# BlaineHeffron/WaveformML

Hardware: AMD Instinct MI355X
Metric: waveforms/sec (LitPSD sparse-conv training step) (higher is better)
Workload: dtype bf16; 1 GPU; SubMConv3d PSD net, 14x11 PMT grid x 256 samples, Cin=2 Cout=32, 256 events/rank/step, rulebook rebuilt every step; active_voxels_per_rank=84164, global_batch=256, parallelism=dp1, execution=hipgraph

## Files before the change

### include/wfsparse.h

```cpp
#ifndef WFSPARSE_H
#define WFSPARSE_H

#include <stddef.h>
#include <stdint.h>

#ifdef __cplusplus
extern "C" {
#endif

#define WFS_OK 0
#define WFS_EINVAL 1
#define WFS_EOVERFLOW 2
#define WFS_EHIP 3
#define WFS_EWORKSPACE 4

#define WFS_F32 0
#define WFS_BF16 1
#define WFS_F16 2

#define WFS_MAX_DIM 4

#define WFS_ABI_VERSION 6
int wfs_abi_version(void);
const char *wfs_last_error(void);
// ... 86 lines not shown
    int32_t transpose;
    float *dW;
} wfs_dw_job;

int wfs_gather_dw(const int32_t *table, const int32_t *kmap_host, int32_t K, int32_t identity_k,
                  int64_t R, const void *S, int32_t Cs, const void *G, int64_t G_rows, int32_t Cg,
                  int32_t swap, float *dW, int32_t dtype, void *workspace, size_t workspace_bytes,
                  const int64_t *r_dev, wfs_dw_job *defer, int32_t packed_kl, void *stream);

int wfs_conv_backward(const int32_t *table, int32_t K, int32_t identity_k, int64_t R, const void *X, const void *dY,
                      int64_t dY_rows, int32_t Cin, int32_t Cout, const float *W, void *dX, float *dW, int32_t dtype,
                      void *workspace, size_t workspace_bytes, const int64_t *r_dev, wfs_dw_job *defer,
                      int32_t packed_kl, void *stream);

int wfs_dw_reduce_jobs(const wfs_dw_job *jobs, int32_t n, void *stream);

size_t wfs_column_sum_workspace_bytes(int32_t C);
int wfs_column_sum(const void *X, int64_t R, int32_t C, float *out, void *workspace, size_t workspace_bytes,
                   int32_t dtype, const int64_t *r_dev, void *stream);

int wfs_scatter_conv(const int32_t *table, int32_t K, int32_t identity_k, int64_t R, const void *X,
                     int32_t Cx, const float *W, int32_t Cw_in, int32_t Cw_out, int32_t transpose_w,
                     float *Y_accum, int32_t dtype, void *stream);

int wfs_maxpool_fwd(const int32_t *table, const int32_t *kmap_host, int32_t K, int64_t R, const void *X, int64_t X_rows,
                    int32_t C, void *Y, int32_t dtype, const int64_t *r_dev, void *stream);
int wfs_maxpool_packed_ok(int32_t packed_kl, int32_t K, int32_t C, int32_t dtype);
int wfs_maxpool_bwd(const int32_t *table, int32_t K, int32_t packed_kl, int64_t N, const void *X, const void *Y,
                    const void *dY, int64_t M_rows, int32_t C, void *dX, int32_t dtype, const int64_t *n_dev, void *stream);

// ... 289 lines not shown
```

### waveformml_amd/_lib.py

```python
import ctypes
import os

import torch

_HERE = os.path.dirname(os.path.abspath(__file__))
LIB_PATH = os.environ.get("WFS_LIB") or os.path.join(_HERE, "lib", "libwfsparse.so")

WFS_OK, WFS_EINVAL, WFS_EOVERFLOW, WFS_EHIP, WFS_EWORKSPACE = 0, 1, 2, 3, 4
WFS_F32, WFS_BF16, WFS_F16 = 0, 1, 2
WFS_TENSOR_TARGET_I64 = 3
WFS_MAX_DIM = 4
WFS_RNN_RELU, WFS_RNN_TANH = 0, 1
WFS_LOSS_L1, WFS_LOSS_MSE = 0, 1
WFS_PREDICT_ROWS_PER_BLOCK = 256
WFS_PREDICT_WAVEFORM, WFS_PREDICT_PULSE = 0, 1
WFS_PREDICT_DENSE, WFS_PREDICT_EVENT, WFS_PREDICT_ROWS = 0, 1, 2
WFS_ABI_VERSION = 6
TIMER_GATHER_CONV, TIMER_GATHER_DW, TIMER_RULEBOOK, TIMER_CONV_BACKWARD = 0, 1, 2, 3

c_i32p = ctypes.POINTER(ctypes.c_int32)
c_i64p = ctypes.POINTER(ctypes.c_int64)
c_f32p = ctypes.POINTER(ctypes.c_float)
_vp, _i32, _i64, _sz = ctypes.c_void_p, ctypes.c_int32, ctypes.c_int64, ctypes.c_size_t
_dbl = ctypes.c_double
# ... 41 lines not shown
    "wfs_wide_linear_ok": (ctypes.c_int, [_i64, _i32, _i32, _i32]),
    "wfs_wide_linear_workspace_bytes": (_sz, [_i64, _i32, _i32, _i32]),
    "wfs_wide_linear_fwd": (ctypes.c_int, [_vp, _i64, _i32, _vp, _vp, _i32, _vp, _i32, _vp, _sz, _vp]),
    "wfs_wide_linear_bwd": (ctypes.c_int, [_vp, _vp, _i64, _i32, _vp, _i32, _vp, _vp, _vp, _i32, _vp, _sz, _vp]),
    "wfs_event_offsets_ints": (_sz, [_i32]),
    "wfs_event_offsets": (ctypes.c_int, [_vp, _i64, _i32, _i32, _vp, _vp, _vp]),
    "wfs_event_rulebook_ok": (ctypes.c_int, [ctypes.POINTER(Geometry)]),
    "wfs_event_rulebook_flag_ints": (_sz, [_i32]),
    "wfs_event_rulebook_subm": (ctypes.c_int, [ctypes.POINTER(Geometry), _vp, _i64, _vp, _vp, _vp, _vp, _vp, _vp]),
    "wfs_gather_dw_workspace_bytes": (_sz, [_i32, _i64, _i32, _i32]),
    "wfs_gather_dw": (ctypes.c_int, [_vp, c_i32p, _i32, _i32, _i64, _vp, _i32, _vp, _i64, _i32, _i32, _vp, _i32, _vp,
                                     _sz, _vp, ctypes.POINTER(DwJob), _i32, _vp]),
    "wfs_conv_backward": (ctypes.c_int, [_vp, _i32, _i32, _i64, _vp, _vp, _i64, _i32, _i32, _vp, _vp, _vp, _i32, _vp, _sz,
                                         _vp, ctypes.POINTER(DwJob), _i32, _vp]),
    "wfs_dw_reduce_jobs": (ctypes.c_int, [ctypes.POINTER(DwJob), _i32, _vp]),
    "wfs_scatter_conv": (ctypes.c_int, [_vp, _i32, _i32, _i64, _vp, _i32, _vp, _i32, _i32, _i32, _vp, _i32, _vp]),
    "wfs_maxpool_fwd": (ctypes.c_int, [_vp, c_i32p, _i32, _i64, _vp, _i64, _i32, _vp, _i32, _vp, _vp]),
    "wfs_maxpool_packed_ok": (ctypes.c_int, [_i32, _i32, _i32, _i32]),
    "wfs_maxpool_bwd": (ctypes.c_int, [_vp, _i32, _i32, _i64, _vp, _vp, _vp, _i64, _i32, _vp, _i32, _vp, _vp]),
    "wfs_bn_workspace_bytes": (_sz, [_i64, _i32]),
    "wfs_column_sum_workspace_bytes": (_sz, [_i32]),
    "wfs_column_sum": (ctypes.c_int, [_vp, _i64, _i32, _vp, _vp, _sz, _i32, _vp, _vp]),
    "wfs_bn_relu_fwd": (ctypes.c_int, [_vp, _i64, _i32, _vp, _vp, _vp, _vp, _vp, ctypes.c_float, ctypes.c_float, _i32,
                                       _i32, _vp, _vp, _vp, _vp, _sz, _i32, _vp, _vp]),
    "wfs_bn_relu_bwd": (ctypes.c_int, [_vp, _vp, _i64, _i32, _vp, _vp, _vp, _vp, _i32, _i32, _vp, _vp, _vp, _vp, _sz,
                                       _i32, _vp, _vp]),
    "wfs_rulebook_cell_map": (ctypes.c_int, [ctypes.POINTER(Geometry), _i64, _vp, ctypes.POINTER(_vp), ctypes.POINTER(_vp),
                                             c_i64p]),
    "wfs_to_dense_mapped": (ctypes.c_int, [_vp, _vp, _vp, _i64, _vp, _i32, _i64, _i32, _vp, _i32, _vp]),
    "wfs_to_dense_bwd_mapped": (ctypes.c_int, [_vp, _vp, _vp, _i64, _vp, _i32, _i64, _i32, _vp, _i32, _vp]),
# ... 192 lines not shown
```

### waveformml_amd/csrc/bn.hip

```cpp
#include "wfs_common.h"

#include <atomic>
#include <cstdlib>
#include <mutex>

namespace {

constexpr int TB = 256;
constexpr int MAXC = 1024;

__device__ __forceinline__ long long valid_rows(long long N, const long long *n_dev) {
    long long v = n_dev ? *n_dev : N;
    return v < N ? v : N;
}

template <typename T, int VEC>
__device__ __forceinline__ void load_vec(const T *p, float *out) {
    if constexpr (VEC == 4 && sizeof(T) == 4) {
        float4 v = *reinterpret_cast<const float4 *>(p);
        out[0] = v.x; out[1] = v.y; out[2] = v.z; out[3] = v.w;
    } else if constexpr (VEC == 4) {
        uint2 v = *reinterpret_cast<const uint2 *>(p);
        wfs_unpack2<T>(v.x, out[0], out[1]);
        wfs_unpack2<T>(v.y, out[2], out[3]);
// ... 964 lines not shown
                                                              (int)nblk, save_mean, save_invstd, gamma, beta,       \
                                                              training, relu, (T *)dX, dgamma, dbeta);              \
    } while (0)
    if (dtype == WFS_F32) {
        if (vec4) WFS_BN_BWD(float, 4); else WFS_BN_BWD(float, 1);
    } else if (dtype == WFS_BF16) {
        if (vec4) WFS_BN_BWD(wfs_bf16, 4); else WFS_BN_BWD(wfs_bf16, 1);
    } else {
        if (vec4) WFS_BN_BWD(wfs_f16, 4); else WFS_BN_BWD(wfs_f16, 1);
    }
#undef WFS_BN_BWD
    WFS_LAUNCH_CHECK();
    return WFS_OK;
}

extern "C" int wfs_bn_relu_bwd(const void *X, const void *dY, int64_t N, int32_t C, const float *gamma,
                               const float *beta, const float *save_mean, const float *save_invstd, int32_t training,
                               int32_t relu, void *dX, float *dgamma, float *dbeta, void *workspace,
                               size_t workspace_bytes, int32_t dtype, const int64_t *n_dev_, void *stream_) {
    hipStream_t stream = (hipStream_t)stream_;
    const long long *n_dev = (const long long *)n_dev_;
    if (bw_ok(N, C) && N > 0 && wfs_dtype_ok(dtype)) {
        WFS_REQUIRE(X && dY && dX && save_mean && save_invstd && workspace, WFS_EINVAL, "NULL device pointer");
        WFS_REQUIRE(workspace_bytes >= wfs_bn_workspace_bytes(N, C), WFS_EWORKSPACE, "workspace too small");
        float *partial = (float *)workspace;
        if (dtype == WFS_F32)
            return bw_bwd<float>(X, dY, N, C, gamma, beta, save_mean, save_invstd, training, relu, dX, dgamma, dbeta,
                                 partial, n_dev, stream);
        if (dtype == WFS_BF16)
            return bw_bwd<wfs_bf16>(X, dY, N, C, gamma, beta, save_mean, save_invstd, training, relu, dX, dgamma, dbeta,
// ... 23 lines not shown
```

### waveformml_amd/csrc/conv_mfma.hip

```cpp
#include <stdlib.h>

#include "wfs_common.h"

namespace {

typedef float f32x16 __attribute__((ext_vector_type(16)));
typedef float f32x4 __attribute__((ext_vector_type(4)));
constexpr int F32_GROUP = 4;

struct KMap {
    int v[128];
};

__device__ __forceinline__ long long valid_rows(long long R, const long long *r_dev) {
    long long v = r_dev ? *r_dev : R;
    return v < R ? v : R;
}

__device__ __forceinline__ int packed_entry(int e, int o) { return (e >= 0 && (e & 7) == o) ? (e >> 3) : -1; }
__device__ __forceinline__ void table_row_of(int pk, int k, int *trow, int *osel) {
    const int kq = pk ? k / pk : k;
    *trow = kq;
    *osel = pk ? k - kq * pk : -1;
}
// ... 1151 lines not shown
            int col = (i & 3) + 8 * (i >> 2) + 4 * h;
            sRed[wid * 1024 + col * 32 + c] = half ? acc1[i] : acc0[i];
        }
        __syncthreads();
        for (int e = threadIdx.x; e < 1024; e += 512) {
            float v = 0.f;
#pragma unroll
            for (int w = 0; w < C2_WAVES; ++w) v += sRed[w * 1024 + e];
            const int ee = half * 1024 + e;
            if (ee < K * 64) part[(long long)blockIdx.x * K * 64 + ee] = v;
        }
        __syncthreads();
    }
}

constexpr int C2F_WAVES = 8;
__global__ void __launch_bounds__(512, 2) k_gdw_c32c2_f32(const int *__restrict__ table, int mirror, int K, int identity_k,
                                                         long long Rcap, const long long *__restrict__ r_dev,
                                                         const float *__restrict__ S, const float *__restrict__ G,
                                                         float *__restrict__ part) {
    __shared__ int sNbT[C2F_WAVES][28 * 33];
    __shared__ float sRed[C2F_WAVES][1024];
    const int lane = threadIdx.x & 63, wid = threadIdx.x >> 6;
    const int c = lane & 31, h = lane >> 5;
    int *myNb = sNbT[wid];
    const long long R = valid_rows(Rcap, r_dev);
    const long long ntiles = (R + 31) >> 5;
    f32x16 acc0, acc1;
#pragma unroll
    for (int i = 0; i < 16; ++i) acc0[i] = acc1[i] = 0.f;
// ... 523 lines not shown
                table, mirror, K, identity_k, R, r_dev, (const wfs_bf16 *)S, (const wfs_bf16 *)G, part);
        else
            k_gdw_c32c2_bf16<wfs_f16><<<dim3((unsigned)chunks), dim3(512), 0, stream>>>(
                table, mirror, K, identity_k, R, r_dev, (const wfs_f16 *)S, (const wfs_f16 *)G, part);
    }
    WFS_LAUNCH_CHECK();
    const long long per = (long long)K * 64;
    if (defer) {
        *defer = wfs_dw_job{part, chunks, per, K, 2, 32, swap ? 0 : 1, dW};
        return WFS_OK;
    }
    k_slab_reduce<<<dim3((unsigned)((per + 31) / 32)), dim3(chunks > 64 ? 1024 : 256), 0, stream>>>(part, chunks, per, K, 2, 32, swap ? 0 : 1, dW);
    WFS_LAUNCH_CHECK();
    return WFS_OK;
}
```

### waveformml_amd/csrc/gather_conv.hip

```cpp
#include "wfs_common.h"

namespace {

constexpr int TB = 256;
constexpr int CT = 8;

struct KMap {
    int v[128];
};

__device__ __forceinline__ long long valid_rows(long long R, const long long *r_dev) {
    long long v = r_dev ? *r_dev : R;
    return v < R ? v : R;
}

template <typename T, bool TRANSPOSE_W>
__global__ void __launch_bounds__(TB) k_gather_conv(const int *__restrict__ table, KMap kmap, int K, int identity_k,
                                                    long long R, const long long *__restrict__ r_dev,
                                                    const T *__restrict__ X, int Cx,
                                                    const float *__restrict__ W, int Cw_in, int Cw_out,
                                                    const float *__restrict__ bias, T *__restrict__ Y, int Cy) {
    const int lane = threadIdx.x & 63;
    const int wid = __builtin_amdgcn_readfirstlane(threadIdx.x >> 6);
    const long long r = (long long)blockIdx.x * 64 + lane;
// ... 546 lines not shown
        int rc = gather_dw_impl(table, nullptr, K, identity_k, R, X, Cin, dY, dY_rows, Cout, 0, dW, dtype, workspace,
                                workspace_bytes, r_dev, defer, stream_, packed_kl);
        if (rc != WFS_OK) return rc;
        return gather_conv_impl(table, nullptr, K, identity_k, R, dY, dY_rows, Cout, W, Cin, Cout, 1, nullptr, dX, dtype, r_dev,
                                stream_, packed_kl);
    }
    WFS_REQUIRE(X && dY && W && workspace, WFS_EINVAL, "NULL device pointer");
    const size_t need = wfs_gather_dw_workspace_bytes(K, R, Cin, Cout);
    WFS_REQUIRE(workspace_bytes >= need, WFS_EWORKSPACE, "workspace %zu < %zu", workspace_bytes, need);
    if (defer) *defer = wfs_dw_job{nullptr, 0, 0, 0, 0, 0, 0, nullptr};
    WfsTimerScope timer(WFS_TIMER_CONV_BACKWARD, stream);
    return wfs_launch_bwd32_h16(table, packed_kl, K, identity_k, R, (const long long *)r_dev, X, dY, W, dX, 0, dW,
                                (float *)workspace, dtype, defer, stream);
}

extern "C" int wfs_dw_reduce_jobs(const wfs_dw_job *jobs, int32_t n, void *stream) {
    WFS_REQUIRE(n >= 0 && n <= 16 && (n == 0 || jobs), WFS_EINVAL, "%d jobs (0 .. 16)", n);
    wfs_dw_job live[16];
    int m = 0;
    for (int i = 0; i < n; ++i) {
        if (jobs[i].nslabs <= 0) continue;
        WFS_REQUIRE(jobs[i].part && jobs[i].dW && jobs[i].per > 0 && jobs[i].A > 0 && jobs[i].B > 0, WFS_EINVAL,
                    "job %d is incomplete", i);
        live[m++] = jobs[i];
    }
    WfsTimerScope timer(WFS_TIMER_GATHER_DW, (hipStream_t)stream);
    return wfs_launch_dw_jobs(live, m, (hipStream_t)stream);
}

namespace {
// ... 59 lines not shown
```

### waveformml_amd/csrc/wfs_common.h

```cpp
#pragma once
#include <hip/hip_runtime.h>
#include <stdint.h>
#include <stdio.h>

#include "../../include/wfsparse.h"

#define WFS_WAVE 64

void wfs_set_error(const char *fmt, ...);

#define WFS_HIP_CHECK(expr)                                                                  \
    do {                                                                                     \
        hipError_t _e = (expr);                                                              \
        if (_e != hipSuccess) {                                                              \
            wfs_set_error("%s failed: %s (%s:%d)", #expr, hipGetErrorString(_e), __FILE__,   \
                          __LINE__);                                                         \
            return WFS_EHIP;                                                                 \
        }                                                                                    \
    } while (0)

#define WFS_LAUNCH_CHECK() WFS_HIP_CHECK(hipGetLastError())

#define WFS_REQUIRE(cond, code, ...)                                                         \
    do {                                                                                     \
// ... 85 lines not shown
int wfs_launch_wide_dw(const int *table, const int *kmap_host, int K, int identity_k, long long R, const long long *r_dev,
                       const void *S, int Cs, const void *G, long long G_rows, int Cg, int swap, float *dW, int dtype,
                       void *workspace, size_t workspace_bytes, hipStream_t stream);
size_t wfs_dw_fast_workspace(int K, long long R, int Cs, int Cg);
int wfs_launch_gdw32(const int *table, int K, int identity_k, long long R, const long long *r_dev, const void *S,
                     const void *G, int swap, float *dW, float *part, int dtype, wfs_dw_job *defer, hipStream_t stream,
                     int packed_kl = 0);
bool wfs_bwd32_fused_ok(int K, int packed_kl, int dtype);
int wfs_launch_bwd32_h16(const int *table, int packed_kl, int K, int identity_k, long long R, const long long *r_dev,
                         const void *S, const void *G, const float *W, void *dX, int swap, float *dW, float *part, int dtype,
                         wfs_dw_job *defer, hipStream_t stream);
int wfs_launch_gdw_c32c2(const int *table, int mirror, int K, int identity_k, long long R, const long long *r_dev,
                         const void *S, const void *G, int swap, float *dW, float *part, int dtype,
                         wfs_dw_job *defer, hipStream_t stream);
int wfs_launch_dw_jobs(const wfs_dw_job *jobs, int n, hipStream_t stream);
```

### waveformml_amd/spconv/conv.py

```python
import math

import numpy as np
import torch
from torch import nn
from torch.nn import init

from . import functional as Fsp
from . import ops
from .modules import SparseModule
from .tensor import IndiceData, SparseConvTensor


class SparseConvolution(SparseModule, ops.StickyFlags):
    def __init__(self, ndim, in_channels, out_channels, kernel_size=3, stride=1, padding=0, dilation=1,
                 groups=1, bias=True, subm=False, output_padding=0, transposed=False, inverse=False,
                 indice_key=None, fused_bn=False, use_hash=False, algo=None):
        super(SparseConvolution, self).__init__()
        assert groups == 1
        self.ndim = ndim
        self.in_channels = in_channels
        self.out_channels = out_channels
        self.kernel_size = ops._listify(kernel_size, ndim)
        self.conv1x1 = int(np.prod(self.kernel_size)) == 1
        self.stride = ops._listify(stride, ndim)
# ... 17 lines not shown
            self.register_parameter('bias', None)
        self.reset_parameters()

    def calibration_count(self):
        if self.subm or self.conv1x1 or self.inverse:
            return None
        return self.last_rulebook.M

    def reset_parameters(self):
        init.kaiming_uniform_(self.weight, a=math.sqrt(5))
        if self.bias is not None:
            fan_in, _ = init._calculate_fan_in_and_fan_out(self.weight)
            bound = 1 / math.sqrt(fan_in)
            init.uniform_(self.bias, -bound, bound)

    def forward(self, input):
        assert isinstance(input, SparseConvTensor)
        features = input.features
        indices = input.indices
        spatial_shape = input.spatial_shape
        batch_size = input.batch_size
        if self.transposed:
            out_spatial_shape = ops.get_deconv_output_size(spatial_shape, self.kernel_size, self.stride,
                                                           self.padding, self.dilation, self.output_padding)
        elif not self.subm:
            out_spatial_shape = ops.get_conv_output_size(spatial_shape, self.kernel_size, self.stride,
                                                         self.padding, self.dilation)
        else:
            out_spatial_shape = spatial_shape
        if self.conv1x1:
            features = Fsp.pointwise_conv(features, self.weight, self.bias, input.n_valid)
            out_tensor = SparseConvTensor(features, input.indices, input.spatial_shape, input.batch_size)
            out_tensor.indice_dict = input.indice_dict
            out_tensor.grid = input.grid
            out_tensor.unique = input.unique
            out_tensor.n_valid = input.n_valid
            out_tensor.prefetched = getattr(input, "prefetched", None)
            return out_tensor
        datas = input.find_indice_pair(self.indice_key)
        if self.inverse:
            assert datas is not None and self.indice_key is not None
            rb = datas.rulebook
            out_spatial_shape = datas.spatial_shape
            assert rb.K == np.prod(self.kernel_size), "inverse conv must have same kernel size as its couple conv"
            out_indices = rb.indices
            out_features = Fsp.indice_inverse_conv(features, self.weight, self.bias, rb)
            out_unique = None if rb.has_dup else True
            out_n_valid = rb.n_dev
        else:
            pre = getattr(input, "prefetched", None)
            if pre is not None and id(self) in pre:
                rb = pre[id(self)]
                if rb.ready is not None:
                    rb.ready.wait()
# ... 4 lines not shown
            elif self.indice_key is not None and datas is not None:
                rb = datas.rulebook
            else:
                rb = ops.build_rulebook(indices, batch_size, spatial_shape, self.kernel_size, self.stride,
                                        self.padding, self.dilation, self.subm, known_unique=input.unique,
                                        n_dev=input.n_valid, out_capacity=getattr(self, "out_capacity", None),
                                        transposed=self.transposed, output_padding=self.output_padding,
                                        events=getattr(input, "events", None), flags=self._sticky_flags(),
                                        want_cell_map=getattr(input, "dense_follows", True))
                if getattr(rb, "events_in", None) is not None:
                    input.events = rb.events_in
                self.last_rulebook = rb
                input.unique = not rb.has_dup
                input.indice_dict[self.indice_key] = IndiceData(rb, spatial_shape)
            out_indices = rb.out_indices
            if self.subm:
                out_features = Fsp.indice_subm_conv(features, self.weight, self.bias, rb)
                out_unique = input.unique
            else:
                out_features = Fsp.indice_conv(features, self.weight, self.bias, rb)
                out_unique = True
            out_n_valid = rb.m_dev
        out_tensor = SparseConvTensor(out_features, out_indices, out_spatial_shape, batch_size)
        out_tensor.indice_dict = input.indice_dict
        out_tensor.grid = input.grid
        out_tensor.unique = out_unique
        out_tensor.n_valid = out_n_valid
        out_tensor.prefetched = getattr(input, "prefetched", None)
        if self.subm:
            out_tensor.events = getattr(input, "events", None)
        elif not self.inverse and getattr(rb, "events_out", None) is not None:
            out_tensor.events = rb.events_out
        if not self.subm and not self.inverse:
            out_tensor.cell_map = getattr(rb, "cell_map", None)
        return out_tensor


def _conv_class(name, ndim, **fixed):
    def __init__(self, in_channels, out_channels, kernel_size, stride=1, padding=0, dilation=1, groups=1,
                 bias=True, indice_key=None, use_hash=False, algo=None):
        SparseConvolution.__init__(self, ndim, in_channels, out_channels, kernel_size, stride, padding, dilation,
                                   groups, bias, indice_key=indice_key, use_hash=use_hash, algo=algo, **fixed)
    return type(name, (SparseConvolution,), {"__init__": __init__, "__module__": __name__})


def _inverse_class(name, ndim):
    def __init__(self, in_channels, out_channels, kernel_size, indice_key=None, bias=True, algo=None):
        SparseConvolution.__init__(self, ndim, in_channels, out_channels, kernel_size, bias=bias, inverse=True,
                                   indice_key=indice_key, algo=algo)
# ... 24 lines not shown
```

### waveformml_amd/spconv/functional.py

```python
import ctypes

import torch
from torch.autograd import Function

from .. import _lib

CONV, SUBM, INVERSE = 0, 1, 2

ACCOUNT = None


def _account(kind, table, R, rows_in, c_in, rows_out, c_out, K, cw_in, cw_out, esize):
    if ACCOUNT is None:
        return
    pairs = int((table >= 0).sum().item()) if table is not None else int(R)
    ACCOUNT.append(dict(kind=kind, pairs=pairs,
                        bytes=rows_in * c_in * esize + rows_out * c_out * esize + pairs * 8 + K * cw_in * cw_out * 4,
                        flops=2 * pairs * cw_in * cw_out))


def _features_ok(t):
    if not t.is_cuda:
        raise RuntimeError("waveformml_amd.spconv: features must be on the GPU (there is no CPU path)")
    return t.contiguous()
# ... 461 lines not shown
            dtype, device = ctx.like
            dY = as_grad(grad_output, dtype)
            dX = torch.empty((M, C), dtype=dtype, device=device)
            _lib.check(lib.wfs_to_dense_bwd_mapped(_lib.ptr(dY), ticket, slot, M, _lib.ptr(ctx.m_dev), batch_size, V, C,
                                                   _lib.ptr(dX), _lib.dtype_code(dX), _lib.stream_ptr()))
            return dX, None, None, None, None, None, None
        (indices,) = ctx.saved_tensors
        dY = grad_output.contiguous()
        dX = _rows((M, C), dY, ctx.m_dev)
        _lib.check(lib.wfs_to_dense_bwd(_lib.ptr(dY), _lib.ptr(indices), M, len(spatial), _lib.i32_array(spatial),
                                        batch_size, C, _lib.ptr(dX), _lib.dtype_code(dY), _lib.ptr(ctx.m_dev),
                                        _lib.stream_ptr()))
        return dX, None, None, None, None, None, None


class BatchNormReLUFunction(Function):

    @staticmethod
    def forward(ctx, x, weight, bias, running_mean, running_var, momentum, eps, training, relu, n_dev=None,
                batches_tracked=None):
        lib = _lib.load()
        x = _features_ok(x)
        N, C = x.shape
        y = _rows(tuple(x.shape), x, n_dev)
        for t in (weight, bias, running_mean, running_var):
            assert t is None or (t.dtype == torch.float32 and t.numel() == C and t.is_contiguous())
        save_mean = torch.empty((C,), dtype=torch.float32, device=x.device)
        save_invstd = torch.empty((C,), dtype=torch.float32, device=x.device)
        ws = torch.empty((max(int(lib.wfs_bn_workspace_bytes(N, C)), 1),), dtype=torch.uint8, device=x.device)
        _lib.check(lib.wfs_bn_relu_fwd(_lib.ptr(x), N, C, _lib.ptr(weight), _lib.ptr(bias), _lib.ptr(running_mean),
                                       _lib.ptr(running_var), _lib.ptr(batches_tracked) if training else None,
                                       float(momentum), float(eps), 1 if training else 0,
                                       1 if relu else 0, _lib.ptr(y), _lib.ptr(save_mean), _lib.ptr(save_invstd),
                                       _lib.ptr(ws), ws.numel(), _lib.dtype_code(x), _lib.ptr(n_dev),
                                       _lib.stream_ptr()))
        ctx.save_for_backward(x, weight, bias, save_mean, save_invstd)
        ctx.flags = (bool(training), bool(relu))
        ctx.n_dev = n_dev
        return y

    @staticmethod
    def backward(ctx, grad_output):
        x, weight, bias, save_mean, save_invstd = ctx.saved_tensors
        training, relu = ctx.flags
        dx, dgamma, dbeta = bn_relu_backward(x, grad_output, weight, bias, save_mean, save_invstd, training, relu, ctx.n_dev)
        return dx, dgamma, dbeta, None, None, None, None, None, None, None, None


def bn_relu_backward(x, grad_output, weight, bias, save_mean, save_invstd, training, relu, n_dev):
    lib = _lib.load()
# ... 13 lines not shown
def batch_norm_relu(features, bn, relu, n_dev=None):
    training = bn.training or (bn.running_mean is None and bn.running_var is None)
    tracked = bn.num_batches_tracked if (bn.training and bn.track_running_stats) else None
    return BatchNormReLUFunction.apply(
        features, bn.weight, bn.bias, bn.running_mean if bn.track_running_stats else None,
        bn.running_var if bn.track_running_stats else None, bn.momentum, bn.eps, training, relu, n_dev, tracked)


def can_fuse_batch_norm(bn, features):
    c = bn.num_features
    return (type(bn) is torch.nn.BatchNorm1d and bn.momentum is not None and features.is_cuda and features.dim() == 2
            and features.dtype in (torch.float32, torch.bfloat16, torch.float16) and features.shape[0] > 0
            and 1 <= c <= 65536
            and (bn.weight is None or bn.weight.dtype == torch.float32)
            and (bn.training or bn.running_mean is not None))


class SkinnyLinearFunction(Function):

    @staticmethod
    def forward(ctx, x, weight, bias):
        lib = _lib.load()
        x = _features_ok(x)
        B, I = x.shape
        O = weight.shape[0]
        w = weight.detach().float().contiguous()
        b = None if bias is None else bias.detach().float().contiguous()
        y = torch.empty((B, O), dtype=torch.float32, device=x.device)
        _lib.check(lib.wfs_head_fwd(_lib.ptr(x), B, I, _lib.ptr(w), _lib.ptr(b), O, _lib.ptr(y), _lib.dtype_code(x),
                                    _lib.stream_ptr()))
# ... 317 lines not shown
```

### waveformml_amd/spconv/modules.py

```python
from collections import OrderedDict

import torch
from torch import nn


class SparseModule(nn.Module):
    pass


def _is_sparse_tensor(x):
    from .tensor import SparseConvTensor
    return isinstance(x, SparseConvTensor)


class _SideJoin(object):

    def __init__(self, side):
        self.event = torch.cuda.Event()
        self.event.record(side)
        self.waited = set()

    def wait(self, stream=None):
        stream = stream if stream is not None else torch.cuda.current_stream()
        key = stream.cuda_stream
# ... 80 lines not shown
                        events = getattr(rb, "events_out", None)
                elif isinstance(m, SparseMaxPool) and not m.subm:
                    rb = ops.build_rulebook(indices, x.batch_size, spatial, m.kernel_size, m.stride, m.padding,
                                            m.dilation, False, known_unique=True, n_dev=n_dev,
                                            out_capacity=getattr(m, "out_capacity", None), events=events,
                                            flags=m._sticky_flags(),
                                            want_cell_map=SparseSequential._dense_follows(mods, at))
                    rb.ready = _SideJoin(side)
                    plan[id(m)] = rb
                    indices, spatial, n_dev = rb.out_indices, rb.out_spatial_shape, rb.m_dev
                    events = getattr(rb, "events_out", None)
                elif isinstance(m, SparseModule):
                    break
        x.prefetched = plan

    def forward(self, input):
        return self.run(input, list(self._modules.values()))

    def run(self, input, mods, stop_before_dense=False):
        from . import functional as Fsp
        from . import ops
        want_prefetch = (ops.PREFETCH_RULEBOOKS and _is_sparse_tensor(input) and input.n_valid is not None
                         and getattr(input, "prefetched", None) is None and input.features.is_cuda)
        i = 0
        while i < len(mods):
            module = mods[i]
            if stop_before_dense and i == len(mods) - 1 and isinstance(module, ToDense) and _is_sparse_tensor(input):
                break
            if isinstance(module, SparseModule):
                if _is_sparse_tensor(input):
                    input.dense_follows = self._dense_follows(mods, i)
                input = module(input)
                if want_prefetch and _is_sparse_tensor(input):
                    want_prefetch = False
                    self._prefetch_rulebooks(mods[i + 1:], input)
            elif _is_sparse_tensor(input):
                if input.indices.shape[0] != 0:
                    if isinstance(module, nn.BatchNorm1d) and Fsp.can_fuse_batch_norm(module, input.features):
                        relu = i + 1 < len(mods) and type(mods[i + 1]) is nn.ReLU
                        input.features = Fsp.batch_norm_relu(input.features, module, relu, input.n_valid)
                        if relu:
                            i += 1
                    else:
                        if input.n_valid is not None and type(module) is not nn.ReLU:
                            raise RuntimeError("device-count (padded) SparseConvTensors only support the fused "
                                               "BatchNorm1d/ReLU pair between sparse layers, got %s" % type(module).__name__)
                        input.features = module(input.features)
# ... 18 lines not shown
```

Baseline: 557,700 events/s.

## Fuse first sparse conv backward with BatchNorm/ReLU backward into one dW kernel

Result: faster. 565,600 events/s (median of 6 runs) (+1.4%).

```diff
diff --git a/include/wfsparse.h b/include/wfsparse.h
--- a/include/wfsparse.h
+++ b/include/wfsparse.h
@@ -124,6 +124,13 @@
                       int32_t packed_kl, void *stream);
 
 int wfs_dw_reduce_jobs(const wfs_dw_job *jobs, int32_t n, void *stream);
+
+size_t wfs_first_conv_bn_backward_workspace_bytes(int32_t K, int64_t R);
+int wfs_first_conv_bn_backward(const int32_t *table, const int32_t *kmap_host, int32_t K, int32_t identity_k, int64_t R,
+                               const void *Z, const void *dY, const void *X, int64_t X_rows, const float *gamma,
+                               const float *beta, const float *save_mean, const float *save_invstd, int32_t relu,
+                               float *dW, float *dgamma, float *dbeta, int32_t dtype, void *workspace,
+                               size_t workspace_bytes, const int64_t *r_dev, wfs_dw_job *defer, void *stream);
 
 size_t wfs_column_sum_workspace_bytes(int32_t C);
 int wfs_column_sum(const void *X, int64_t R, int32_t C, float *out, void *workspace, size_t workspace_bytes,
diff --git a/waveformml_amd/_lib.py b/waveformml_amd/_lib.py
--- a/waveformml_amd/_lib.py
+++ b/waveformml_amd/_lib.py
@@ -79,6 +79,9 @@
     "wfs_conv_backward": (ctypes.c_int, [_vp, _i32, _i32, _i64, _vp, _vp, _i64, _i32, _i32, _vp, _vp, _vp, _i32, _vp, _sz,
                                          _vp, ctypes.POINTER(DwJob), _i32, _vp]),
     "wfs_dw_reduce_jobs": (ctypes.c_int, [ctypes.POINTER(DwJob), _i32, _vp]),
+    "wfs_first_conv_bn_backward_workspace_bytes": (_sz, [_i32, _i64]),
+    "wfs_first_conv_bn_backward": (ctypes.c_int, [_vp, c_i32p, _i32, _i32, _i64, _vp, _vp, _vp, _i64, _vp, _vp, _vp, _vp,
+                                                  _i32, _vp, _vp, _vp, _i32, _vp, _sz, _vp, ctypes.POINTER(DwJob), _vp]),
     "wfs_scatter_conv": (ctypes.c_int, [_vp, _i32, _i32, _i64, _vp, _i32, _vp, _i32, _i32, _i32, _vp, _i32, _vp]),
     "wfs_maxpool_fwd": (ctypes.c_int, [_vp, c_i32p, _i32, _i64, _vp, _i64, _i32, _vp, _i32, _vp, _vp]),
     "wfs_maxpool_packed_ok": (ctypes.c_int, [_i32, _i32, _i32, _i32]),
diff --git a/waveformml_amd/csrc/bn.hip b/waveformml_amd/csrc/bn.hip
--- a/waveformml_amd/csrc/bn.hip
+++ b/waveformml_amd/csrc/bn.hip
@@ -1002,6 +1002,42 @@
     return WFS_OK;
 }
 
+int wfs_launch_bn_bwd_reduce(const void *X, const void *dY, long long N, int C, const float *gamma, const float *beta,
+                             const float *save_mean, const float *save_invstd, int relu, float *partial, int dtype,
+                             const long long *n_dev, hipStream_t stream, int *nblk_out) {
+    const dim3 block(TB);
+    long long rb = 0;
+    const int per = rr_plan(N, C, dtype == WFS_F32 ? 8 : 16, &rb);
+    if (per) {
+        const dim3 g2((unsigned)rb);
+#define WFS_BN_RED_RR(T, PER)                                                                                          \
+    k_bn_reduce_rr<T, PER, 1><<<g2, block, 0, stream>>>((const T *)X, (const T *)dY, N, n_dev, C, save_mean,           \
+                                                         save_invstd, gamma, beta, relu, partial)
+#define WFS_BN_RED_RR_T(T)                                                                                             \
+    if (per == 2) WFS_BN_RED_RR(T, 2); else if (per == 4) WFS_BN_RED_RR(T, 4); else if (per == 8) WFS_BN_RED_RR(T, 8);   \
+    else WFS_BN_RED_RR(T, 16)
+        if (dtype == WFS_F32) { WFS_BN_RED_RR_T(float); } else if (dtype == WFS_BF16) { WFS_BN_RED_RR_T(wfs_bf16); } else { WFS_BN_RED_RR_T(wfs_f16); }
+#undef WFS_BN_RED_RR_T
+#undef WFS_BN_RED_RR
+        *nblk_out = (int)rb;
+    } else {
+        const long long nblk = bn_reduce_blocks(N, C), rpb = wfs_cdiv(N, nblk);
+        const dim3 grid((unsigned)nblk);
+        if (dtype == WFS_F32)
+            k_bn_reduce<float, 4, 1><<<grid, block, 0, stream>>>((const float *)X, (const float *)dY, N, n_dev, C, C, rpb,
+                                                                 save_mean, save_invstd, gamma, beta, relu, partial);
+        else if (dtype == WFS_BF16)
+            k_bn_reduce<wfs_bf16, 4, 1><<<grid, block, 0, stream>>>((const wfs_bf16 *)X, (const wfs_bf16 *)dY, N, n_dev, C, C,
+                                                                    rpb, save_mean, save_invstd, gamma, beta, relu, partial);
+        else
+            k_bn_reduce<wfs_f16, 4, 1><<<grid, block, 0, stream>>>((const wfs_f16 *)X, (const wfs_f16 *)dY, N, n_dev, C, C,
+                                                                   rpb, save_mean, save_invstd, gamma, beta, relu, partial);
+        *nblk_out = (int)nblk;
+    }
+    WFS_LAUNCH_CHECK();
+    return WFS_OK;
+}
+
 extern "C" int wfs_bn_relu_bwd(const void *X, const void *dY, int64_t N, int32_t C, const float *gamma,
                                const float *beta, const float *save_mean, const float *save_invstd, int32_t training,
                                int32_t relu, void *dX, float *dgamma, float *dbeta, void *workspace,
diff --git a/waveformml_amd/csrc/conv_mfma.hip b/waveformml_amd/csrc/conv_mfma.hip
--- a/waveformml_amd/csrc/conv_mfma.hip
+++ b/waveformml_amd/csrc/conv_mfma.hip
@@ -1189,6 +1189,176 @@
     }
 }
 
+template <typename H>
+__global__ void __launch_bounds__(512, 2) k_gdw_bnapply_c32c2(const int *__restrict__ table, int mirror, int K,
+                                                             int identity_k, long long Rcap,
+                                                             const long long *__restrict__ r_dev,
+                                                             const H *__restrict__ Z, const H *__restrict__ S,
+                                                             const H *__restrict__ G, const float *__restrict__ partial,
+                                                             int nblk, const float *__restrict__ mean,
+                                                             const float *__restrict__ invstd,
+                                                             const float *__restrict__ gamma, const float *__restrict__ beta,
+                                                             int relu, float *__restrict__ dgamma, float *__restrict__ dbeta,
+                                                             float *__restrict__ part) {
+    __shared__ __attribute__((aligned(16))) unsigned sA[C2_WAVES][32 * 33];
+    __shared__ __attribute__((aligned(16))) unsigned short sB[C2_WAVES][32 * 32];
+    __shared__ float sSlice[2 * 256];
+    __shared__ float4 sP[32], sQ[32];
+    const int lane = threadIdx.x & 63, wid = threadIdx.x >> 6;
+    const int c = lane & 31, h = lane >> 5;
+    const int grow = lane >> 2, gchunk = lane & 3;
+    unsigned *myA = sA[wid];
+    unsigned short *myB = sB[wid];
+    const long long R = valid_rows(Rcap, r_dev);
+    {
+        const int col = threadIdx.x & 31, sl = (threadIdx.x >> 5) & 7;
+        if (threadIdx.x < 256) {
+            float av[32], bv[32];
+#pragma unroll
+            for (int i = 0; i < 32; ++i) {
+                const int p = sl + i * 8;
+                const float *q = partial + (long long)(p < nblk ? p : 0) * 64 + col;
+                av[i] = q[0];
+                bv[i] = q[32];
+            }
+            float a = 0.f, bb = 0.f;
+#pragma unroll
+            for (int i = 0; i < 32; ++i) {
+                const bool ok = sl + i * 8 < nblk;
+                a += ok ? av[i] : 0.f;
+                bb += ok ? bv[i] : 0.f;
+            }
+            sSlice[threadIdx.x] = a;
+            sSlice[256 + threadIdx.x] = bb;
+        }
+        __syncthreads();
+        if (threadIdx.x < 32) {
+            float ta = 0.f, tb = 0.f;
+            for (int q = 0; q < 8; ++q) {
+                ta += sSlice[q * 32 + col];
+                tb += sSlice[256 + q * 32 + col];
+            }
+            if (blockIdx.x == 0) {
+                if (dbeta) dbeta[col] = ta;
+                if (dgamma) dgamma[col] = tb;
+            }
+            const float invN = R > 0 ? 1.f / (float)R : 0.f;
+            sP[col] = make_float4(mean[col], invstd[col], gamma ? gamma[col] : 1.f, beta ? beta[col] : 0.f);
+            sQ[col] = make_float4(ta * invN, tb * invN, 0.f, 0.f);
+        }
+        __syncthreads();
+    }
+    const long long ntiles = (R + 31) >> 5;
+    f32x16 acc0, acc1;
+#pragma unroll
+    for (int i = 0; i < 16; ++i) acc0[i] = acc1[i] = 0.f;
+    const unsigned *Gw = reinterpret_cast<const unsigned *>(G);
+    for (long long tile = (long long)blockIdx.x * C2_WAVES + wid; tile < ntiles; tile += (long long)gridDim.x * C2_WAVES) {
+        const long long row0 = tile * 32;
+        const long long trow = row0 + c < R ? row0 + c : R - 1;
+        const bool tlive = row0 + c < R;
+        int nb[14];
+#pragma unroll
+        for (int t = 0; t < 14; ++t) {
+            int k = 2 * t + h;
+            int kk = k < K ? k : K - 1;
+            nb[t] = table[(long long)(mirror ? K - 1 - kk : kk) * Rcap + trow];
+        }
+        const long long ra = row0 + grow, rb = row0 + grow + 16;
+        const long long oa = (ra < R ? ra : R - 1) * 32 + gchunk * 8, ob = (rb < R ? rb : R - 1) * 32 + gchunk * 8;
+        const uint4 s0 = *(const uint4 *)(S + oa);
+        const uint4 s1 = *(const uint4 *)(S + ob);
+        const uint4 z0 = *(const uint4 *)(Z + oa);
+        const uint4 z1 = *(const uint4 *)(Z + ob);
+        unsigned xv[14];
+#pragma unroll
+        for (int t = 0; t < 14; ++t) {
+            int k = 2 * t + h;
+            int n = (k == identity_k) ? (int)trow : nb[t];
+            bool ok = tlive && k < K && n >= 0;
+            nb[t] = ok ? n : -1;
+            xv[t] = Gw[ok ? n : 0];
+        }
+        __builtin_amdgcn_wave_barrier();
+        {
+            const unsigned zw[2][4] = {{z0.x, z0.y, z0.z, z0.w}, {z1.x, z1.y, z1.z, z1.w}};
+            const unsigned gw[2][4] = {{s0.x, s0.y, s0.z, s0.w}, {s1.x, s1.y, s1.z, s1.w}};
+            unsigned ow[2][4];
+#pragma unroll
+            for (int j = 0; j < 4; ++j) {
+                const float4 pl = sP[gchunk * 8 + 2 * j], ph = sP[gchunk * 8 + 2 * j + 1];
+                const float4 ql = sQ[gchunk * 8 + 2 * j], qh = sQ[gchunk * 8 + 2 * j + 1];
+#pragma unroll
+                for (int half = 0; half < 2; ++half) {
+                    float xv2[2], gv2[2], o[2];
+                    wfs_unpack2<H>(zw[half][j], xv2[0], xv2[1]);
+                    wfs_unpack2<H>(gw[half][j], gv2[0], gv2[1]);
+#pragma unroll
+                    for (int e = 0; e < 2; ++e) {
+                        const float m = e ? ph.x : pl.x, is = e ? ph.y : pl.y, ga = e ? ph.z : pl.z, be = e ? ph.w : pl.w;
+                        const float k1 = e ? qh.x : ql.x, k2 = e ? qh.y : ql.y;
+                        float xh = (xv2[e] - m) * is;
+                        float gi = gv2[e];
+                        if (relu && !(fmaf(ga, xh, be) > 0.f)) gi = 0.f;
+                        o[e] = ga * is * (gi - k1 - xh * k2);
+                    }
+                    ow[half][j] = wfs_pack2<H>(o[0], o[1]);
+                }
+            }
+            *(uint4 *)(myB + grow * 32 + gchunk * 8) = keep_if(make_uint4(ow[0][0], ow[0][1], ow[0][2], ow[0][3]), ra < R);
+            *(uint4 *)(myB + (grow + 16) * 32 + gchunk * 8) = keep_if(make_uint4(ow[1][0], ow[1][1], ow[1][2], ow[1][3]), rb < R);
+        }
+#pragma unroll
+        for (int t = 0; t < 14; ++t) {
+            int k = 2 * t + h;
+            myA[c * 33 + k] = nb[t] >= 0 ? xv[t] : 0u;
+        }
+        if (h == 0) {
+#pragma unroll
+            for (int k = 28; k < 32; ++k) myA[c * 33 + k] = 0u;
+        }
+        __builtin_amdgcn_wave_barrier();
+        const unsigned short *A16 = reinterpret_cast<const unsigned short *>(myA);
+        unsigned wa[2][2][4], wb[2][4];
+#pragma unroll
+        for (int st = 0; st < 2; ++st)
+#pragma unroll
+            for (int m = 0; m < 4; ++m) {
+                int r0 = 16 * st + 8 * h + 2 * m;
+                wa[0][st][m] = (unsigned)A16[r0 * 66 + c] | ((unsigned)A16[(r0 + 1) * 66 + c] << 16);
+                wa[1][st][m] = (unsigned)A16[r0 * 66 + 32 + c] | ((unsigned)A16[(r0 + 1) * 66 + 32 + c] << 16);
+                wb[st][m] = (unsigned)myB[r0 * 32 + c] | ((unsigned)myB[(r0 + 1) * 32 + c] << 16);
+            }
+#pragma unroll
+        for (int st = 0; st < 2; ++st) {
+            uint4 a_lo = {wa[0][st][0], wa[0][st][1], wa[0][st][2], wa[0][st][3]};
+            uint4 a_hi = {wa[1][st][0], wa[1][st][1], wa[1][st][2], wa[1][st][3]};
+            uint4 bb = {wb[st][0], wb[st][1], wb[st][2], wb[st][3]};
+            acc0 = mfma16<H>(a_lo, bb, acc0);
+            acc1 = mfma16<H>(a_hi, bb, acc1);
+        }
+    }
+    __syncthreads();
+    float *sRed = reinterpret_cast<float *>(&sA[0][0]);
+#pragma unroll
+    for (int half = 0; half < 2; ++half) {
+#pragma unroll
+        for (int i = 0; i < 16; ++i) {
+            int col = (i & 3) + 8 * (i >> 2) + 4 * h;
+            sRed[wid * 1024 + col * 32 + c] = half ? acc1[i] : acc0[i];
+        }
+        __syncthreads();
+        for (int e = threadIdx.x; e < 1024; e += 512) {
+            float v = 0.f;
+#pragma unroll
+            for (int w = 0; w < C2_WAVES; ++w) v += sRed[w * 1024 + e];
+            const int ee = half * 1024 + e;
+            if (ee < K * 64) part[(long long)blockIdx.x * K * 64 + ee] = v;
+        }
+        __syncthreads();
+    }
+}
+
 constexpr int C2F_WAVES = 8;
 __global__ void __launch_bounds__(512, 2) k_gdw_c32c2_f32(const int *__restrict__ table, int mirror, int K, int identity_k,
                                                          long long Rcap, const long long *__restrict__ r_dev,
@@ -1742,3 +1912,33 @@
     WFS_LAUNCH_CHECK();
     return WFS_OK;
 }
+
+long long wfs_first_bn_slabs(long long R) {
+    const long long ntiles = (R + 31) >> 5;
+    long long chunks = (ntiles + C2_WAVES - 1) / C2_WAVES;
+    return chunks > 512 ? 512 : (chunks < 1 ? 1 : chunks);
+}
+
+int wfs_launch_first_bn_bwd(const int *table, int mirror, int K, int identity_k, long long R, const long long *r_dev,
+                            const void *Z, const void *dY, const void *X, const float *gamma, const float *beta,
+                            const float *mean, const float *invstd, int relu, const float *partial, int nblk, float *dW,
+                            float *dgamma, float *dbeta, float *part, int dtype, wfs_dw_job *defer, hipStream_t stream) {
+    const long long chunks = wfs_first_bn_slabs(R);
+    if (dtype == WFS_BF16)
+        k_gdw_bnapply_c32c2<wfs_bf16><<<dim3((unsigned)chunks), dim3(512), 0, stream>>>(
+            table, mirror, K, identity_k, R, r_dev, (const wfs_bf16 *)Z, (const wfs_bf16 *)dY, (const wfs_bf16 *)X, partial,
+            nblk, mean, invstd, gamma, beta, relu, dgamma, dbeta, part);
+    else
+        k_gdw_bnapply_c32c2<wfs_f16><<<dim3((unsigned)chunks), dim3(512), 0, stream>>>(
+            table, mirror, K, identity_k, R, r_dev, (const wfs_f16 *)Z, (const wfs_f16 *)dY, (const wfs_f16 *)X, partial,
+            nblk, mean, invstd, gamma, beta, relu, dgamma, dbeta, part);
+    WFS_LAUNCH_CHECK();
+    const long long per = (long long)K * 64;
+    if (defer) {
+        *defer = wfs_dw_job{part, chunks, per, K, 2, 32, 0, dW};
+        return WFS_OK;
+    }
+    k_slab_reduce<<<dim3((unsigned)((per + 31) / 32)), dim3(chunks > 64 ? 1024 : 256), 0, stream>>>(part, chunks, per, K, 2, 32, 0, dW);
+    WFS_LAUNCH_CHECK();
+    return WFS_OK;
+}
diff --git a/waveformml_amd/csrc/gather_conv.hip b/waveformml_amd/csrc/gather_conv.hip
--- a/waveformml_amd/csrc/gather_conv.hip
+++ b/waveformml_amd/csrc/gather_conv.hip
@@ -584,6 +584,52 @@
                                 (float *)workspace, dtype, defer, stream);
 }
 
+static size_t first_bn_slab_bytes(int32_t K, int64_t R) {
+    return wfs_align_up((size_t)wfs_first_bn_slabs(R) * (size_t)K * 64 * sizeof(float), 256);
+}
+extern "C" size_t wfs_first_conv_bn_backward_workspace_bytes(int32_t K, int64_t R) {
+    return first_bn_slab_bytes(K, R) + wfs_bn_workspace_bytes(R, 32);
+}
+
+extern "C" int wfs_first_conv_bn_backward(const int32_t *table, const int32_t *kmap_host, int32_t K, int32_t identity_k,
+                                          int64_t R, const void *Z, const void *dY, const void *X, int64_t X_rows,
+                                          const float *gamma, const float *beta, const float *save_mean,
+                                          const float *save_invstd, int32_t relu, float *dW, float *dgamma, float *dbeta,
+                                          int32_t dtype, void *workspace, size_t workspace_bytes, const int64_t *r_dev,
+                                          wfs_dw_job *defer, void *stream_) {
+    hipStream_t stream = (hipStream_t)stream_;
+    WFS_REQUIRE(K >= 1 && K <= 27, WFS_EINVAL, "K = %d (1 .. 27)", K);
+    WFS_REQUIRE(dtype == WFS_BF16 || dtype == WFS_F16, WFS_EINVAL, "16-bit rows only (dtype %d)", dtype);
+    WFS_REQUIRE(dW, WFS_EINVAL, "NULL dW");
+    WFS_REQUIRE(R >= 0 && R < (1ll << 31) && X_rows < (1ll << 31), WFS_EINVAL, "too many rows");
+    if (defer) *defer = wfs_dw_job{nullptr, 0, 0, 0, 0, 0, 0, nullptr};
+    if (R == 0) {
+        WFS_HIP_CHECK(hipMemsetAsync(dW, 0, (size_t)K * 64 * sizeof(float), stream));
+        if (dgamma) WFS_HIP_CHECK(hipMemsetAsync(dgamma, 0, 32 * sizeof(float), stream));
+        if (dbeta) WFS_HIP_CHECK(hipMemsetAsync(dbeta, 0, 32 * sizeof(float), stream));
+        return WFS_OK;
+    }
+    WFS_REQUIRE(table && Z && dY && X && save_mean && save_invstd && workspace, WFS_EINVAL, "NULL device pointer");
+    WFS_REQUIRE(((uintptr_t)workspace & 15) == 0, WFS_EINVAL, "the workspace must be 16-byte aligned");
+    WFS_REQUIRE(workspace_bytes >= wfs_first_conv_bn_backward_workspace_bytes(K, R), WFS_EWORKSPACE, "workspace too small");
+    bool is_ident = true, is_mirror = kmap_host != nullptr;
+    for (int k = 0; k < K && kmap_host; ++k) {
+        is_ident = is_ident && kmap_host[k] == k;
+        is_mirror = is_mirror && kmap_host[k] == K - 1 - k;
+    }
+    WFS_REQUIRE(is_ident || is_mirror, WFS_EINVAL, "the column map must be the identity or the SubM mirror");
+    float *part = (float *)workspace;
+    float *partial = (float *)((char *)workspace + first_bn_slab_bytes(K, R));
+    int nblk = 0;
+    int rc = wfs_launch_bn_bwd_reduce(Z, dY, R, 32, gamma, beta, save_mean, save_invstd, relu ? 1 : 0, partial, dtype,
+                                      (const long long *)r_dev, stream, &nblk);
+    if (rc != WFS_OK) return rc;
+    WfsTimerScope timer(WFS_TIMER_GATHER_DW, stream);
+    return wfs_launch_first_bn_bwd(table, is_ident ? 0 : 1, K, identity_k, R, (const long long *)r_dev, Z, dY, X, gamma, beta,
+                                   save_mean, save_invstd, relu ? 1 : 0, partial, nblk, dW, dgamma, dbeta, part, dtype, defer,
+                                   stream);
+}
+
 extern "C" int wfs_dw_reduce_jobs(const wfs_dw_job *jobs, int32_t n, void *stream) {
     WFS_REQUIRE(n >= 0 && n <= 16 && (n == 0 || jobs), WFS_EINVAL, "%d jobs (0 .. 16)", n);
     wfs_dw_job live[16];
diff --git a/waveformml_amd/csrc/wfs_common.h b/waveformml_amd/csrc/wfs_common.h
--- a/waveformml_amd/csrc/wfs_common.h
+++ b/waveformml_amd/csrc/wfs_common.h
@@ -123,3 +123,11 @@
                          const void *S, const void *G, int swap, float *dW, float *part, int dtype,
                          wfs_dw_job *defer, hipStream_t stream);
 int wfs_launch_dw_jobs(const wfs_dw_job *jobs, int n, hipStream_t stream);
+int wfs_launch_bn_bwd_reduce(const void *X, const void *dY, long long N, int C, const float *gamma, const float *beta,
+                             const float *save_mean, const float *save_invstd, int relu, float *partial, int dtype,
+                             const long long *n_dev, hipStream_t stream, int *nblk_out);
+long long wfs_first_bn_slabs(long long R);
+int wfs_launch_first_bn_bwd(const int *table, int mirror, int K, int identity_k, long long R, const long long *r_dev,
+                            const void *Z, const void *dY, const void *X, const float *gamma, const float *beta,
+                            const float *mean, const float *invstd, int relu, const float *partial, int nblk, float *dW,
+                            float *dgamma, float *dbeta, float *part, int dtype, wfs_dw_job *defer, hipStream_t stream);
diff --git a/waveformml_amd/spconv/conv.py b/waveformml_amd/spconv/conv.py
--- a/waveformml_amd/spconv/conv.py
+++ b/waveformml_amd/spconv/conv.py
@@ -55,7 +55,7 @@
             bound = 1 / math.sqrt(fan_in)
             init.uniform_(self.bias, -bound, bound)
 
-    def forward(self, input):
+    def forward(self, input, bn_tail=None):
         assert isinstance(input, SparseConvTensor)
         features = input.features
         indices = input.indices
@@ -79,6 +79,7 @@
             out_tensor.prefetched = getattr(input, "prefetched", None)
             return out_tensor
         datas = input.find_indice_pair(self.indice_key)
+        fused = False
         if self.inverse:
             assert datas is not None and self.indice_key is not None
             rb = datas.rulebook
@@ -113,7 +114,12 @@
                 input.unique = not rb.has_dup
                 input.indice_dict[self.indice_key] = IndiceData(rb, spatial_shape)
             out_indices = rb.out_indices
-            if self.subm:
+            fused = (bn_tail is not None and not self.transposed
+                     and Fsp.first_conv_bn_ok(features, self.weight, self.bias, rb, bn_tail[0]))
+            if fused:
+                out_features = features
+                out_unique = input.unique if self.subm else True
+            elif self.subm:
                 out_features = Fsp.indice_subm_conv(features, self.weight, self.bias, rb)
                 out_unique = input.unique
             else:
@@ -132,6 +138,11 @@
             out_tensor.events = rb.events_out
         if not self.subm and not self.inverse:
             out_tensor.cell_map = getattr(rb, "cell_map", None)
+        if not self.inverse and fused:
+            bn, relu, between = bn_tail
+            out_tensor.features = Fsp.first_conv_bn_relu(features, self.weight, rb, bn, relu,
+                                                         None if between is None else (lambda: between(out_tensor)))
+            out_tensor.bn_applied = True
         return out_tensor
 
 
diff --git a/waveformml_amd/spconv/functional.py b/waveformml_amd/spconv/functional.py
--- a/waveformml_amd/spconv/functional.py
+++ b/waveformml_amd/spconv/functional.py
@@ -499,26 +499,32 @@
         return dX, None, None, None, None, None, None
 
 
+def _bn_relu_forward(x, weight, bias, running_mean, running_var, momentum, eps, training, relu, n_dev, batches_tracked):
+    lib = _lib.load()
+    N, C = x.shape
+    y = _rows(tuple(x.shape), x, n_dev)
+    for t in (weight, bias, running_mean, running_var):
+        assert t is None or (t.dtype == torch.float32 and t.numel() == C and t.is_contiguous())
+    save_mean = torch.empty((C,), dtype=torch.float32, device=x.device)
+    save_invstd = torch.empty((C,), dtype=torch.float32, device=x.device)
+    ws = torch.empty((max(int(lib.wfs_bn_workspace_bytes(N, C)), 1),), dtype=torch.uint8, device=x.device)
+    _lib.check(lib.wfs_bn_relu_fwd(_lib.ptr(x), N, C, _lib.ptr(weight), _lib.ptr(bias), _lib.ptr(running_mean),
+                                   _lib.ptr(running_var), _lib.ptr(batches_tracked) if training else None,
+                                   float(momentum), float(eps), 1 if training else 0,
+                                   1 if relu else 0, _lib.ptr(y), _lib.ptr(save_mean), _lib.ptr(save_invstd),
+                                   _lib.ptr(ws), ws.numel(), _lib.dtype_code(x), _lib.ptr(n_dev),
+                                   _lib.stream_ptr()))
+    return y, save_mean, save_invstd
+
+
 class BatchNormReLUFunction(Function):
 
     @staticmethod
     def forward(ctx, x, weight, bias, running_mean, running_var, momentum, eps, training, relu, n_dev=None,
                 batches_tracked=None):
-        lib = _lib.load()
         x = _features_ok(x)
-        N, C = x.shape
-        y = _rows(tuple(x.shape), x, n_dev)
-        for t in (weight, bias, running_mean, running_var):
-            assert t is None or (t.dtype == torch.float32 and t.numel() == C and t.is_contiguous())
-        save_mean = torch.empty((C,), dtype=torch.float32, device=x.device)
-        save_invstd = torch.empty((C,), dtype=torch.float32, device=x.device)
-        ws = torch.empty((max(int(lib.wfs_bn_workspace_bytes(N, C)), 1),), dtype=torch.uint8, device=x.device)
-        _lib.check(lib.wfs_bn_relu_fwd(_lib.ptr(x), N, C, _lib.ptr(weight), _lib.ptr(bias), _lib.ptr(running_mean),
-                                       _lib.ptr(running_var), _lib.ptr(batches_tracked) if training else None,
-                                       float(momentum), float(eps), 1 if training else 0,
-                                       1 if relu else 0, _lib.ptr(y), _lib.ptr(save_mean), _lib.ptr(save_invstd),
-                                       _lib.ptr(ws), ws.numel(), _lib.dtype_code(x), _lib.ptr(n_dev),
-                                       _lib.stream_ptr()))
+        y, save_mean, save_invstd = _bn_relu_forward(x, weight, bias, running_mean, running_var, momentum, eps, training,
+                                                     relu, n_dev, batches_tracked)
         ctx.save_for_backward(x, weight, bias, save_mean, save_invstd)
         ctx.flags = (bool(training), bool(relu))
         ctx.n_dev = n_dev
@@ -562,6 +568,81 @@
             and 1 <= c <= 65536
             and (bn.weight is None or bn.weight.dtype == torch.float32)
             and (bn.training or bn.running_mean is not None))
+
+
+def first_conv_bn_backward(table, kmap, K, identity_k, R, z, dY, features, gamma, beta, save_mean, save_invstd, relu,
+                           r_dev, filters):
+    lib = _lib.load()
+    dW = grad_like(filters, (K, 2, 32)) if filters.numel() == K * 64 else torch.empty((K, 2, 32), dtype=torch.float32,
+                                                                                      device=z.device)
+    dgamma = grad_like(gamma) if gamma is not None else None
+    dbeta = grad_like(beta) if beta is not None else None
+    assert z.dtype == dY.dtype == features.dtype and z.shape == dY.shape == (R, 32) and features.shape[1] == 2
+    assert table.dtype == torch.int32 and table.shape == (K, R)
+    ws = torch.empty((int(lib.wfs_first_conv_bn_backward_workspace_bytes(K, R)),), dtype=torch.uint8, device=z.device)
+    job = _dw_job(dW)
+    _lib.check(lib.wfs_first_conv_bn_backward(_lib.ptr(table), kmap, K, identity_k, R, _lib.ptr(z), _lib.ptr(dY),
+                                              _lib.ptr(features), features.shape[0], _lib.ptr(gamma), _lib.ptr(beta),
+                                              _lib.ptr(save_mean), _lib.ptr(save_invstd), 1 if relu else 0, _lib.ptr(dW),
+                                              _lib.ptr(dgamma), _lib.ptr(dbeta), _lib.dtype_code(z), _lib.ptr(ws),
+                                              ws.numel(), _lib.ptr(r_dev), job, _lib.stream_ptr()))
+    _queue_dw_job(job, ws)
+    if ACCOUNT is not None:
+        _account("gather_dw", table, R, R, 32, features.shape[0], 2, K, 32, 2, z.element_size())
+    return dW, dgamma, dbeta
+
+
+def first_conv_bn_ok(features, filters, conv_bias, rulebook, bn):
+    rb = rulebook
+    return bool(features.is_cuda and features.dim() == 2 and features.shape[1] == 2 and filters.shape[-2] == 2
+                and filters.shape[-1] == 32 and filters.dtype == torch.float32 and rb.K <= 27 and not rb.has_dup
+                and conv_bias is None and features.dtype in (torch.bfloat16, torch.float16)
+                and not features.requires_grad and bn.num_features == 32 and features.shape[0] > 0 and rb.M > 0
+                and (bn.training or (bn.running_mean is None and bn.running_var is None))
+                and type(bn) is torch.nn.BatchNorm1d and bn.momentum is not None
+                and (bn.weight is None or bn.weight.dtype == torch.float32))
+
+
+class FirstConvBNFunction(Function):
+
+    @staticmethod
+    def forward(ctx, features, filters, weight, bias, running_mean, running_var, momentum, eps, relu, rulebook,
+                batches_tracked, between):
+        rb = rulebook
+        features = _features_ok(features)
+        K = rb.K
+        W = filters.detach().reshape(K, 2, 32).float().contiguous()
+        ident = rb.centre_k if rb.subm else -1
+        assert features.shape[0] == rb.N
+        table, kmap = rb.table_by_out()
+        z = gather_conv(table, kmap, K, ident, rb.M, features, W, False, None, rb.m_dev, None)
+        if between is not None:
+            between()
+        y, save_mean, save_invstd = _bn_relu_forward(z, weight, bias, running_mean, running_var, momentum, eps, True,
+                                                     relu, rb.m_dev, batches_tracked)
+        ctx.save_for_backward(features, filters, weight, bias, z, save_mean, save_invstd)
+        ctx.rb, ctx.relu = rb, bool(relu)
+        return y
+
+    @staticmethod
+    def backward(ctx, grad_output):
+        features, filters, weight, bias, z, save_mean, save_invstd = ctx.saved_tensors
+        rb = ctx.rb
+        dY = as_grad(grad_output, z.dtype)
+        table, kmap = rb.table_by_out()
+        dW, dgamma, dbeta = first_conv_bn_backward(table, kmap, rb.K, rb.centre_k if rb.subm else -1, rb.M, z, dY,
+                                                   features, weight, bias, save_mean, save_invstd, ctx.relu, rb.m_dev,
+                                                   filters)
+        dW = dW.reshape(filters.shape).to(filters.dtype)
+        return (None, dW if ctx.needs_input_grad[1] else None, dgamma if ctx.needs_input_grad[2] else None,
+                dbeta if ctx.needs_input_grad[3] else None, None, None, None, None, None, None, None, None)
+
+
+def first_conv_bn_relu(features, filters, rulebook, bn, relu, between=None):
+    tracked = bn.num_batches_tracked if (bn.training and bn.track_running_stats) else None
+    return FirstConvBNFunction.apply(
+        features, filters, bn.weight, bn.bias, bn.running_mean if bn.track_running_stats else None,
+        bn.running_var if bn.track_running_stats else None, bn.momentum, bn.eps, relu, rulebook, tracked, between)
 
 
 class SkinnyLinearFunction(Function):
diff --git a/waveformml_amd/spconv/modules.py b/waveformml_amd/spconv/modules.py
--- a/waveformml_amd/spconv/modules.py
+++ b/waveformml_amd/spconv/modules.py
@@ -118,6 +118,22 @@
                     break
         x.prefetched = plan
 
+    def _bn_tail(self, mods, i, input, want_prefetch):
+        from . import functional as Fsp
+        from .conv import SparseConvolution
+        module = mods[i]
+        if not (isinstance(module, SparseConvolution) and _is_sparse_tensor(input) and i + 1 < len(mods)
+                and isinstance(mods[i + 1], nn.BatchNorm1d) and input.indices.shape[0] != 0
+                and module.in_channels == 2 and module.out_channels == 32 and module.bias is None
+                and not (module.conv1x1 or module.inverse or module.transposed)
+                and torch.is_tensor(input.features) and input.features.is_cuda
+                and input.features.dtype in (torch.bfloat16, torch.float16) and not input.features.requires_grad):
+            return None
+        relu = i + 2 < len(mods) and type(mods[i + 2]) is nn.ReLU
+        rest = mods[i + 1:]
+        between = (lambda out: self._prefetch_rulebooks(rest, out)) if want_prefetch else None
+        return mods[i + 1], relu, between
+
     def forward(self, input):
         return self.run(input, list(self._modules.values()))
 
@@ -134,7 +150,15 @@
             if isinstance(module, SparseModule):
                 if _is_sparse_tensor(input):
                     input.dense_follows = self._dense_follows(mods, i)
-                input = module(input)
+                bn_tail = self._bn_tail(mods, i, input, want_prefetch)
+                if bn_tail is not None:
+                    input = module(input, bn_tail=bn_tail)
+                    if getattr(input, "bn_applied", False):
+                        input.bn_applied = False
+                        want_prefetch = want_prefetch and getattr(input, "prefetched", None) is None
+                        i += 2 if bn_tail[1] else 1
+                else:
+                    input = module(input)
                 if want_prefetch and _is_sparse_tensor(input):
                     want_prefetch = False
                     self._prefetch_rulebooks(mods[i + 1:], input)
```
